# big-nacho/patolette

Hardware: AMD Instinct MI355X
Metric: Mpixels/sec quantized (256-color ICtCp + KMeans) at 1 GPU; palette ΔE vs ref (higher is better)
Workload: dtype f64

## Files before the change

include/patolette_amd.h:

```cpp
#ifndef PATOLETTE_AMD_H
#define PATOLETTE_AMD_H

#include <stddef.h>
#include <stdint.h>

#include "patolette.h"

#ifdef __cplusplus
extern "C" {
#endif

int  patolette_amd_device_count(void);
int  patolette_amd_set_device(int ordinal);
const char *patolette_amd_last_error(void);
void *patolette_amd_malloc(size_t bytes);
void patolette_amd_free(void *dptr);
int  patolette_amd_memcpy_h2d(void *dst, const void *src, size_t bytes);
int  patolette_amd_memcpy_d2h(void *dst, const void *src, size_t bytes);
int  patolette_amd_synchronize(void);
void patolette_amd_release_workspace(void);
int  patolette_amd_fill_image(double *d_planar, size_t n, uint64_t seed);
int  patolette_amd_fill_weights(double *d_weights, size_t n, uint64_t seed);

void patolette_amd_device(size_t width, size_t height, const double *d_data, const double *d_weights,
// ... 155 lines not shown
} patolette_amd__Comm;
void patolette_amd_slice(size_t total_pixels, size_t slice_begin, size_t slice_pixels, const double *slice_data,
                         const double *slice_weights, size_t palette_size, const patolette__QuantizationOptions *options,
                         const patolette_amd__Comm *comm, double *palette, size_t *slice_map, int *exit_code);
void patolette_amd_slice_device(size_t total_pixels, size_t slice_begin, size_t slice_pixels, const double *d_slice_data,
                                const double *d_slice_weights, size_t palette_size, const patolette__QuantizationOptions *options,
                                const patolette_amd__Comm *comm, double *palette, void *d_slice_map, int map_elem_bytes,
                                int *exit_code);
int patolette_amd_set_invariant_sums(int on);
int patolette_amd_set_kmeans_update(int mode);

int patolette_amd_set_split_loop(int mode);
int patolette_amd_set_global_quantiser(int on_device);

int patolette_amd_set_subsample_cache(int on);

int patolette_amd_subsample_indices(size_t n, size_t take, int32_t *out);
int patolette_amd_eigen_sym3(const double a_colmajor[9], double w[3], double z[9]);
int patolette_amd_principal_axis(const double cov6[6], double axis[3]);
int patolette_amd_eigen_sym3_device(const double *a_colmajor, size_t count, double *w, double *z, int *info);
int patolette_amd_debug_gq_table(const double *table, const uint32_t *counts, int weighted, size_t palette_size, int route, int *kbase, int *error,
                                 int *cuts, unsigned char *bucket_table, uint64_t *begin, uint64_t *n, double *sw, double *mean,
                                 uint64_t *prefix_w0, double *prefix, int *cut_table);
int patolette_amd_pow(const double *x, double y, double *out, size_t n);

enum {
    PAMD_SRGB_TO_ICTCP = 0,
    PAMD_SRGB_TO_CIELUV = 1,
    PAMD_ICTCP_TO_REC2020 = 2,
    PAMD_CIELUV_TO_REC2020 = 3,
    PAMD_SRGB_TO_REC2020 = 4,
    PAMD_REC2020_TO_SRGB = 5,
    PAMD_CIELUV_TO_ICTCP = 6
};
int patolette_amd_convert(int which, double *planar, size_t n);

int patolette_amd_quantize_clusters(const double *colors, const double *weights, size_t n, size_t K,
                                    double *centers, size_t *n_clusters);

int patolette_amd_kmeans_refine(const double *colors, const double *weights, size_t n,
                                double *centers_io, size_t k, int niter, size_t max_samples);
int patolette_amd_debug_km_route(void);

int patolette_amd_nn_map(const double *colors, size_t n, const double *palette, size_t k, size_t *map);
int patolette_amd_debug_nn_route(int route);
int patolette_amd_debug_nn_map_elem(const double *colors, size_t n, const double *palette, size_t k, int map_elem_bytes, int misalign,
// ... 66 lines not shown
```

patolette_amd/_native.py:

```python
import ctypes as C
import os

HERE = os.path.dirname(os.path.abspath(__file__))
LIB_PATH = os.path.join(HERE, "lib", "libpatolette_amd.so")

dp = C.POINTER(C.c_double)
zp = C.POINTER(C.c_size_t)


class QuantizationOptions(C.Structure):
    _fields_ = [("dither", C.c_bool), ("palette_only", C.c_bool), ("color_space", C.c_int),
                ("kmeans_niter", C.c_int), ("kmeans_max_samples", C.c_size_t), ("verbose", C.c_bool)]


class Stats(C.Structure):
    _fields_ = [(n, C.c_double) for n in ("ms_total", "ms_upload", "ms_convert", "ms_gq", "ms_lq",
                                          "ms_kmeans", "ms_map", "ms_download", "ms_saliency")] + \
               [(n, C.c_size_t) for n in ("n_base_clusters", "n_clusters", "split_evals", "split_px",
                                          "lq_rounds", "kmeans_samples", "dither_segments", "dither_repairs",
                                          "dither_rounds", "dither_through", "dither_jumps", "dither_solo")]

    def as_dict(self):
        return {n: getattr(self, n) for n, _ in self._fields_}

# ... 32 lines not shown
    "patolette_amd_last_error": (C.c_char_p, []),
    "patolette_amd_malloc": (C.c_void_p, [C.c_size_t]),
    "patolette_amd_free": (None, [C.c_void_p]),
    "patolette_amd_memcpy_h2d": (C.c_int, [C.c_void_p, C.c_void_p, C.c_size_t]),
    "patolette_amd_memcpy_d2h": (C.c_int, [C.c_void_p, C.c_void_p, C.c_size_t]),
    "patolette_amd_synchronize": (C.c_int, []),
    "patolette_amd_release_workspace": (None, []),
    "patolette_amd_batch_dmap": (None, [C.c_size_t, C.c_size_t, C.c_size_t, C.POINTER(C.c_void_p), C.c_int, C.POINTER(dp), C.c_double,
                                        C.c_size_t, C.POINTER(QuantizationOptions), C.POINTER(dp), C.c_void_p, C.c_int,
                                        C.POINTER(C.c_int)]),
    "patolette_amd_slice": (None, [C.c_size_t, C.c_size_t, C.c_size_t, dp, dp, C.c_size_t, C.POINTER(QuantizationOptions),
                                   C.POINTER(Comm), dp, zp, C.POINTER(C.c_int)]),
    "patolette_amd_slice_device": (None, [C.c_size_t, C.c_size_t, C.c_size_t, C.c_void_p, C.c_void_p, C.c_size_t,
                                          C.POINTER(QuantizationOptions), C.POINTER(Comm), dp, C.c_void_p, C.c_int, C.POINTER(C.c_int)]),
    "patolette_amd_set_invariant_sums": (C.c_int, [C.c_int]),
    "patolette_amd_set_kmeans_update": (C.c_int, [C.c_int]),
    "patolette_amd_set_subsample_cache": (C.c_int, [C.c_int]),
    "patolette_amd_subsample_indices": (C.c_int, [C.c_size_t, C.c_size_t, C.POINTER(C.c_int32)]),
    "patolette_amd_eigen_sym3": (C.c_int, [dp, dp, dp]),
    "patolette_amd_principal_axis": (C.c_int, [dp, dp]),
    "patolette_amd_eigen_sym3_device": (C.c_int, [dp, C.c_size_t, dp, dp, C.POINTER(C.c_int)]),
    "patolette_amd_debug_gq_table": (C.c_int, [dp, C.c_void_p, C.c_int, C.c_size_t, C.c_int, C.POINTER(C.c_int), C.POINTER(C.c_int), C.c_void_p,
                                               C.c_void_p, C.c_void_p, C.c_void_p, dp, dp, C.c_void_p, dp, C.c_void_p]),
    "patolette_amd_fill_image": (C.c_int, [C.c_void_p, C.c_size_t, C.c_uint64]),
    "patolette_amd_fill_weights": (C.c_int, [C.c_void_p, C.c_size_t, C.c_uint64]),
    "patolette_amd_device": (None, [C.c_size_t, C.c_size_t, C.c_void_p, C.c_void_p, C.c_size_t,
                                    C.POINTER(QuantizationOptions), dp, C.c_void_p, C.c_int, C.POINTER(C.c_int)]),
    "patolette_amd_quantize": (None, [C.c_size_t, C.c_size_t, dp, dp, C.c_double, C.c_size_t, C.POINTER(QuantizationOptions), dp, zp,
                                      C.POINTER(C.c_int)]),
    "patolette_amd_quantize_rows": (None, [C.c_size_t, C.c_size_t, dp, dp, C.c_double, C.c_size_t, C.POINTER(QuantizationOptions), dp,
                                           zp, C.POINTER(C.c_int)]),
    "patolette_amd_saliency_weights": (C.c_int, [C.c_size_t, C.c_size_t, dp, C.c_double, dp]),
    "patolette_amd_mbd": (C.c_int, [C.c_size_t, C.c_size_t, C.POINTER(C.c_float), C.c_int, C.POINTER(C.c_float)]),
    **_pair("patolette_amd_u8", None, [C.c_size_t, C.c_size_t, C.c_void_p, C.c_int, C.c_void_p, C.c_double, C.c_size_t,
                                       C.POINTER(QuantizationOptions), dp, C.c_void_p, C.c_void_p, C.c_int, C.c_void_p, C.POINTER(C.c_int)]),
    **_pair("patolette_amd_frames_u8", None, [C.c_size_t, C.c_size_t, C.c_size_t, C.c_void_p, C.c_int, C.c_void_p, C.c_double, C.c_size_t,
                                              C.POINTER(QuantizationOptions), dp, C.c_void_p, C.c_void_p, C.c_int, C.c_void_p,
                                              C.POINTER(C.c_int)]),
    **_pair("patolette_amd_remap_u8", None, [C.c_size_t, C.c_size_t, C.c_size_t, C.c_void_p, C.c_int, dp, C.c_void_p, C.c_size_t, C.c_int,
                                             C.c_void_p, C.c_int, C.c_void_p, C.POINTER(C.c_int)]),
    **_pair("patolette_amd_remap_ordered_u8", None, [C.c_size_t, C.c_size_t, C.c_size_t, C.c_void_p, C.c_int, dp, C.c_void_p, C.c_size_t,
                                                     C.c_double, C.c_void_p, C.c_int, C.c_void_p, C.POINTER(C.c_int)]),
    "patolette_amd_debug_remap_two_pass": (C.c_int, [C.c_int]),
    **_pair("patolette_amd_remap_rgba_u8", None, [C.c_size_t, C.c_size_t, C.c_size_t, C.c_void_p, C.c_int, dp, C.c_void_p, C.c_size_t, C.c_int,
                                                  C.c_int, C.c_double, C.c_void_p, C.c_int, C.c_void_p, C.POINTER(C.c_int)]),
    "patolette_amd_debug_rgba_stamp_quad": (C.c_int, [C.c_int]),
# ... 87 lines not shown
def last_error():
    return lib().patolette_amd_last_error().decode("utf-8", "replace")


def last_stats():
    s = Stats()
    lib().patolette_amd_last_stats(C.byref(s))
    return s.as_dict()


def last_split_trace():
    hdr = SplitTrace()
    n = lib().patolette_amd_last_split_trace(C.byref(hdr), None, 0)
    recs = (SplitRecord * max(1, n))()
    lib().patolette_amd_last_split_trace(C.byref(hdr), recs, n)
    return dict(n_base=hdr.n_base, n_clusters=hdr.n_clusters, stopped_early=bool(hdr.stopped_early),
                gq_axis=[float(v) for v in hdr.gq_axis], gq_cov6=[float(v) for v in hdr.gq_cov6],
                gq_cuts=[int(v) for v in hdr.gq_cuts][:hdr.n_base + 1],
                splits=[dict(row=r.row, new_row=r.new_row, split=r.split, degenerate=r.degenerate, n=r.n, n_left=r.n_left,
                             n_right=r.n_right, sw=r.sw, axis=[float(v) for v in r.axis], cov6=[float(v) for v in r.cov6],
                             dist=r.dist, dist_left=r.dist_left, dist_right=r.dist_right, benefit=r.benefit) for r in recs[:n]])


def debug_gq_table(table, counts, weighted, palette_size, route, details=True):
    import numpy as np
    nq = 14 if weighted else 10
    t = np.ascontiguousarray(table, dtype=np.float64).reshape(-1)
    c = np.ascontiguousarray(counts, dtype=np.uint32).reshape(-1)
    if t.size != nq * 2 * 512 or c.size != 512:
        raise ValueError("debug_gq_table: table must hold %d x 2 x 512 doubles and counts 512 entries" % nq)
    kbase, error = C.c_int(0), C.c_int(0)
    cuts = np.zeros(14, dtype=np.int32)
    lut = np.zeros(512, dtype=np.uint8)
    begin, n = np.zeros(12, dtype=np.uint64), np.zeros(12, dtype=np.uint64)
    sw, mean = np.zeros(12), np.zeros((12, 3))
    pw0 = np.zeros((2, 513), dtype=np.uint64) if details else None
    pre = np.zeros((14, 513)) if details else None
    ctab = np.zeros((13, 513), dtype=np.int32) if details else None
    vp = lambda a: a.ctypes.data_as(C.c_void_p) if a is not None else None
    rc = lib().patolette_amd_debug_gq_table(t.ctypes.data_as(dp), vp(c), 1 if weighted else 0, int(palette_size), int(route), C.byref(kbase),
                                            C.byref(error), vp(cuts), vp(lut), vp(begin), vp(n), sw.ctypes.data_as(dp), mean.ctypes.data_as(dp),
                                            vp(pw0), pre.ctypes.data_as(dp) if details else None, vp(ctab))
    if rc != 0:
        raise RuntimeError("patolette_amd_debug_gq_table: %d (%s)" % (rc, last_error()))
    k = kbase.value
    out = dict(kbase=k, error=error.value, cuts=[int(v) for v in cuts[:k + 1]] if k else [], bucket_table=lut, begin=begin[:k].copy(),
# ... 32 lines not shown
```

patolette_amd/csrc/pipeline.hip:

```cpp
#include <algorithm>
#include <functional>
#include <chrono>
#include <cmath>
#include <atomic>
#include <memory>
#include <mutex>
#include <thread>
#include <future>
#include <type_traits>

#include "color_device.h"
#include "common.h"
#include "host_math.h"
#include "kmeans.h"
#include "map.h"
#include "ordered.h"
#include "delta.h"
#include "measure.h"
#include "lzw.h"
#include "lzw_near.h"
#include "hist.h"
#include "saliency.h"
#include "quant.h"
#include "rgba.h"
// ... 818 lines not shown

struct Engine {
    int device = -1;
    hipStream_t stream = nullptr;
    const Shard *shard = nullptr;
    bool invariant = false;
    DevBuf<unsigned char> commbuf;
    PinBuf<unsigned char> h_comm;
    DevBuf<int> shard_ids;
    PinBuf<float> h_cent;
    PinBuf<ConvertStats> h_cstats;
    hipEvent_t ev_stats = nullptr;
    hipStream_t stream2 = nullptr;
    hipEvent_t ev_up[2] = {nullptr, nullptr}, ev_join = nullptr;
    size_t prep_N = 0, prep_planes = 0;
    DevBuf<double> src, wsrc, cvt, bufA, bufB, aux;
    DevBuf<unsigned short> bkt;
    DevBuf<NodeDev> nodes;
    DevBuf<NodeIn> stage_in;
    DevBuf<NodeOut> stage_out;
    DevBuf<int> ids, round_nodes, node_tile0;
    DevBuf<Tile> tilesA, tilesP;
    DevBuf<double> hist, sum6, dpal;
    DevBuf<unsigned long long> hsize, tileoff;
    DevBuf<unsigned int> hcount, tilecnt;
    DevBuf<unsigned char> lut, dmap, src8, pal8, quant8;
    DevBuf<unsigned char> dl_maps, dl_shown;
    DevBuf<unsigned long long> dl_words, dl_masks;
    DevBuf<unsigned long long> ms_words;
    DevBuf<MeasureTile> ms_tiles;
    DevBuf<unsigned> ms_p8;
    DevBuf<LzwFrame> lz_frames;
    DevBuf<unsigned> lz_stage, lz_bits, lz_out;
    DevBuf<unsigned long long> lz_gbit, lz_words;
    DevBuf<unsigned char> lz_near;
    DevBuf<unsigned> rgba_cnt;
    DevBuf<int> rgba_cpos;
    DevBuf<unsigned char> rgba_rgb, rgba_map;
    DevBuf<double> rgba_w;
    PinBuf<unsigned> h_rgba_m;
    DevBuf<unsigned> rr_words;
    PinBuf<unsigned> h_rr_words;
    DevBuf<unsigned long long> hs_units, hs_words, hs_counts;
    DevBuf<unsigned> hs_tiles;
    DevBuf<unsigned char> hs_rgb;
    DevBuf<double> hs_w;
// ... 279 lines not shown
    E.hist.reserve(z.hist, file, line); E.hsize.reserve(z.hsize, file, line); E.hcount.reserve(z.hcount, file, line); E.lut.reserve(z.lut, file, line);
}

static void gq_prepare(Engine &E, size_t N, bool weighted) {
    hipStream_t s = E.stream;
    const size_t planes = weighted ? 4 : 3;
    const QuantSizes z(N, planes, 1);
    reserve_quant_tables(E, z);
    const int ntA = (int)z.tilesA, ntP = (int)z.tilesP;
    E.h_round.reserve(kBuckets);
    E.round_nodes.reserve(1); E.node_tile0.reserve(2);
    const size_t hs = hist_slot_doubles();
    hipLaunchKernelGGL(k_gq_prepare, 64, 256, 0, s, E.tilesA.p, ntA, E.tilesP.p, ntP, (unsigned long long)N, E.round_nodes.p, E.node_tile0.p,
                       E.hist.p, (unsigned long long)hs, E.hsize.p, E.hcount.p);
    HIP_CHECK(hipGetLastError());
    E.prep_N = N; E.prep_planes = planes;
}



std::atomic<int> g_lq_device{getenv("PAMD_LQ_DEVICE") ? atoi(getenv("PAMD_LQ_DEVICE")) : 2};
std::atomic<int> g_gq_device{getenv("PAMD_GQ_DEVICE") ? atoi(getenv("PAMD_GQ_DEVICE")) : 1};
constexpr size_t kLqDeviceAutoPixels = (size_t)40 << 20;

static bool lq_device_eligible(const Engine &E, size_t N, size_t K, bool verbose, bool allow_device) {
    const int lq_mode = g_lq_device.load(std::memory_order_relaxed);
    return allow_device && (lq_mode == 1 || (lq_mode == 2 && N < kLqDeviceAutoPixels)) && !E.shard && !verbose && K <= (size_t)kLqDevMaxK;
}

static void ws_prepare(Engine &E, size_t N, size_t K, bool weighted, bool verbose) {
    const size_t planes = weighted ? 4 : 3;
    const bool lq_dev = lq_device_eligible(E, N, K, verbose, true);
    E.cvt.reserve(planes * N); E.cstats.reserve(1);
    reserve_quant_tables(E, QuantSizes(N, planes, lq_dev ? (size_t)kLqRoundCap : 1));
    E.round_nodes.reserve(1); E.node_tile0.reserve(2); E.h_round.reserve(kBuckets);
    E.nodes.reserve(std::max<size_t>(4 * K + 64, lq_dev ? (size_t)kLqNodeCap : 0));
    E.h_dbl.reserve(16 * kBuckets * 2 + 64);
    E.gq.reserve(1); E.gqout.reserve(1); E.h_gqout.reserve(1); E.h_gq.reserve(1);
    const size_t nput = kGqMaxK + 1;
    E.stage_in.reserve(nput); E.stage_out.reserve(nput); E.ids.reserve(nput); E.h_stage_in.reserve(nput); E.h_stage_out.reserve(nput);
    E.h_ids.reserve(nput); E.h_ids_get.reserve(nput);
    E.h_cent.reserve(3 * K);
    E.dpal.reserve(3 * K); E.h_pal.reserve(3 * K);
    if (lq_dev) { E.lqctl.reserve(1); E.h_lqhead.reserve(1); E.h_lqrec.reserve(kLqNodeCap); E.h_lqcen.reserve(kLqNodeCap); }
}

// ... 201 lines not shown
    }
}

static bool gq_root_histogram(QuantCall &C) {
    Engine &E = C.E;
    hipStream_t s = E.stream;
    const HNode &root = C.hn[0];
    if (!node_axis(root, C.axis)) return false;
    E.trace.clear();
    E.trace_pending = false;
    E.trace_hdr = patolette_amd__SplitTrace{};
    for (int j = 0; j < 3; j++) E.trace_hdr.gq_axis[j] = C.axis[j];
    for (int q = 0; q < 6; q++) E.trace_hdr.gq_cov6[q] = root.cov6[q] / root.sw;
    {
        NodeIn d = make_nodedev(root, C.bnd);
        for (int j = 0; j < 3; j++) d.axis[j] = C.axis[j];
        d.slot = 0;
        put_nodes(E, {0}, {d});
    }
    launch_minmax(C.qroot, E.tilesA.p, C.ntA0, C.N, E.nodes.p, s, C.mom_path);
    if (C.sh) shard_exchange_keys(E, shard_upload_ids(E, {0}), 1);
    launch_hist(C.qroot, true, E.tilesA.p, C.ntA0, C.N, E.nodes.p, E.hist.p, E.hsize.p, E.hcount.p, s, !C.mom_path, C.Nt >= ((size_t)1 << 18));
    if (C.sh) { comm_sum_dev(E, E.hist.p, C.hs, 0); comm_sum_dev(E, E.hcount.p, kBuckets, 2); }
    return true;
}

static void gq_trace_header(Engine &E) {
    const GqOut &o = *E.h_gqout.p;
    E.trace_hdr.n_base = o.kbase;
    for (int j = 0; j <= o.kbase && j < 14; j++) E.trace_hdr.gq_cuts[j] = (size_t)o.cuts[j];
}

static int finish_device_loop(QuantCall &C, int kbase, int first_base, int nnodes) {
    Engine &E = C.E;
    if (kbase >= 0) E.stats.n_base_clusters = (size_t)kbase;
    E.stats.ms_gq = now_ms() - C.t0;
    C.t0 = now_ms();
    const int rc = lq_device_loop(E, C.N, C.K, C.weighted, C.inv_sums, C.bnd, C.qlq, kbase, first_base, nnodes, C.centers, C.len, C.max_members);
    if (kbase < 0) {
        gq_trace_header(E);
        E.stats.n_base_clusters = (size_t)E.h_gqout.p->kbase;
    }
    if (rc != 0) return rc;
    E.stats.n_clusters = C.len;
    E.trace_hdr.n_clusters = (int32_t)C.len; E.trace_hdr.n_records = (int32_t)E.lq_commits.size();
    E.cluster_centers = C.centers;
// ... 2657 lines not shown
}

int patolette_amd_debug_fault(int which) { return g_debug_fault.exchange(which); }
int patolette_amd_debug_workspace(int flags) { return g_debug_ws.exchange(flags & (kWsPoison | kWsCount | kWsLog)); }
unsigned long long patolette_amd_debug_late_growths(void) { return g_late_growths.load(); }
int patolette_amd_set_split_loop(int mode) { return g_lq_device.exchange(mode < 0 || mode > 2 ? 2 : mode); }
int patolette_amd_set_global_quantiser(int on_device) { return g_gq_device.exchange(on_device ? 1 : 0); }
void patolette_amd_dither_config(int segments, int warm) { dither_config(segments, warm); }
void patolette_amd_dither_layout(int lanes) { dither_layout(lanes); }
int patolette_amd_debug_dither_solo_cap(int cap) { return dither_solo_cap(cap); }
int patolette_amd_debug_dither_stall_passes(int n) { return dither_stall_passes(n); }
int patolette_amd_dither_layout_in_use(size_t width, size_t height, size_t k) { return dither_lane_layout(width, height, (int)k) ? 1 : 0; }
int patolette_amd_debug_dither_lane_tables(double *geom30, float *amb3, unsigned char *tables, size_t capacity) {
    return guarded([&](Engine &E) -> int { return dither_lane_tables(E.nn, geom30, amb3, tables, capacity, E.stream); });
}
void patolette_amd_last_stats(patolette_amd__Stats *out) { *out = engine().stats; }
size_t patolette_amd_last_split_trace(patolette_amd__SplitTrace *hdr, patolette_amd__SplitRecord *recs, size_t capacity) {
    Engine &E = engine();
    try { materialise_trace(E); } catch (const std::exception &e) { E.last_error = e.what(); E.trace.clear(); }
    if (hdr) *hdr = E.trace_hdr;
    if (recs) std::memcpy(recs, E.trace.data(), sizeof *recs * std::min(capacity, E.trace.size()));
    return E.trace.size();
}
size_t patolette_amd_last_cluster_centers(double *out, size_t capacity_rows) {
    Engine &E = engine();
    const size_t len = E.cluster_centers.size() / 3;
    if (out && len <= capacity_rows)
        for (int j = 0; j < 3; j++) for (size_t i = 0; i < len; i++) out[(size_t)j * capacity_rows + i] = E.cluster_centers[(size_t)j * len + i];
    return len;
}
size_t patolette_amd_last_map_palette(double *out, size_t capacity_rows) {
    const std::vector<double> &mp = engine().map_palette;
    const size_t len = mp.size() / 3;
    if (out && capacity_rows >= len)
        for (int j = 0; j < 3; j++) for (size_t i = 0; i < len; i++) out[(size_t)j * capacity_rows + i] = mp[(size_t)j * len + i];
    return len;
}

void patolette_amd_profile_enable(int on) {
    KernelTimer &t = ktimer();
    if (engine().stream) (void)hipStreamSynchronize(engine().stream);
    t.reset();
    t.enabled = on != 0;
}
void patolette_amd_profile_only(const char *kernel_name) { ktimer().only = kernel_name ? kernel_name : ""; ktimer().only_seen = 0; }
void patolette_amd_profile_sample(int period) { ktimer().sample_period = period > 1 ? (unsigned)period : 1u; }
// ... 13 lines not shown
```

patolette_amd/csrc/quant.hip:

```cpp
#include "quant.h"

#include <atomic>

#include <type_traits>

namespace pamd {

template <typename T>
__device__ __forceinline__ T block_scan_incl(T v, T *smem) {
    const int lane = threadIdx.x & 63, wid = threadIdx.x >> 6, nw = blockDim.x >> 6;
#pragma unroll
    for (int o = 1; o < 64; o <<= 1) {
        T t = __shfl_up(v, o, 64);
        if (lane >= o) v += t;
    }
    __syncthreads();
    if (lane == 63) smem[wid] = v;
    __syncthreads();
    if (wid == 0) {
        T s = lane < nw ? smem[lane] : T(0);
#pragma unroll
        for (int o = 1; o < 16; o <<= 1) {
            T t = __shfl_up(s, o, 64);
            if (lane >= o) s += t;
// ... 104 lines not shown
            mn = fmin(mn, d); mx = fmax(mx, d);
        }
    }
    for (; i < t.count; i += 256) {
        size_t p = t.start + i;
        double d = project(px[p], py[p], pz[p], a0, a1, a2);
        mn = fmin(mn, d); mx = fmax(mx, d);
    }
#pragma unroll
    for (int o = 32; o > 0; o >>= 1) { mn = fmin(mn, __shfl_down(mn, o, 64)); mx = fmax(mx, __shfl_down(mx, o, 64)); }
    __shared__ double smn[4], smx[4];
    if ((threadIdx.x & 63) == 0) { smn[threadIdx.x >> 6] = mn; smx[threadIdx.x >> 6] = mx; }
    __syncthreads();
    if (threadIdx.x == 0) {
        for (int w = 1; w < 4; w++) { mn = fmin(mn, smn[w]); mx = fmax(mx, smx[w]); }
        if (mn <= mx) {
            atomicMin(&nd.minkey[blockIdx.x & (kSlots - 1)], f64_key(mn));
            atomicMax(&nd.maxkey[blockIdx.x & (kSlots - 1)], f64_key(mx));
        }
    }
}

constexpr int kHistCombineMin = 12;
template <bool W, bool GQ>
__global__ __launch_bounds__(512) void k_hist(QuantBuffers qb, const Tile *__restrict__ tiles, int ntiles, NodeDev *nodes,
                                              double *hist, unsigned long long *hsize, unsigned int *hcount, const int from_end,
                                              const RoundDyn *__restrict__ dyn) {
    constexpr int NQ = GQ ? (W ? 14 : 10) : (W ? 4 : 3);
    int nblk = (int)gridDim.x;
    if (dyn) {
        ntiles = dyn->ntA;
        nblk = min(ntiles, nblk);
        if ((int)blockIdx.x >= nblk) return;
    }
    constexpr int NQS = GQ ? kNQ_GQ : kNQ_LQ;
    extern __shared__ double lds[];
    double *h = lds;
    unsigned long long *siz = (unsigned long long *)(h + NQ * 2 * kBuckets);
    unsigned int *cnt = (unsigned int *)(siz + kBuckets);
    for (int i = threadIdx.x; i < NQ * 2 * kBuckets; i += blockDim.x) h[i] = 0.0;
    for (int i = threadIdx.x; i < kBuckets; i += blockDim.x) { cnt[i] = 0u; siz[i] = 0ULL; }
    __syncthreads();

    const int per = (ntiles + nblk - 1) / nblk;
    const int bid = from_end ? nblk - 1 - (int)blockIdx.x : (int)blockIdx.x;
    const int tfirst = bid * per, tlast = min(ntiles, tfirst + per);
// ... 107 lines not shown
    const int e1 = (int)((__double_as_longlong(k.M1) >> 52) & 0x7ff) - 1023 - 52;
    const int B = e0 - e1, E = e0 + B;
    const int F = 2 * B < 45 ? 2 * B : 45;
    FixK f;
    f.magic = ldexp(1.5, 52 + E - F); f.s = F - B; f.ghi = ldexp(1.0, e0); f.glo = ldexp(1.0, E - F);
    return f;
}
__device__ __forceinline__ long long fix_quant(const double v, const double magic) {
    return __double_as_longlong(v + magic) - __double_as_longlong(magic);
}
template <bool W, bool GQ>
__global__ __launch_bounds__(512) void k_hist_fix(QuantBuffers qb, const Tile *__restrict__ tiles, int ntiles, NodeDev *nodes,
                                              double *hist, unsigned long long *hsize, unsigned int *hcount, const int from_end) {
    constexpr int NQ = GQ ? (W ? 14 : 10) : (W ? 4 : 3);
    constexpr int NQS = GQ ? kNQ_GQ : kNQ_LQ;
    extern __shared__ unsigned long long lds64[];
    unsigned long long *h = lds64;
    unsigned long long *siz = h + NQ * kBuckets;
    unsigned int *cnt = (unsigned int *)(siz + kBuckets);
    for (int i = threadIdx.x; i < NQ * kBuckets; i += blockDim.x) h[i] = 0ULL;
    for (int i = threadIdx.x; i < kBuckets; i += blockDim.x) { cnt[i] = 0u; siz[i] = 0ULL; }
    __syncthreads();

    const int per = (ntiles + (int)gridDim.x - 1) / (int)gridDim.x;
    const int bid = from_end ? (int)gridDim.x - 1 - (int)blockIdx.x : (int)blockIdx.x;
    const int tfirst = bid * per, tlast = min(ntiles, tfirst + per);
    int since_flush = 0;
    for (int ti = tfirst; ti < tlast; ti++) {
        const Tile t = tiles[ti];
        NodeDev &nd = nodes[t.node];
        const double a0 = nd.axis[0], a1 = nd.axis[1], a2 = nd.axis[2];
        double mn, mx;
        node_minmax(nd, mn, mx);
        const bool degenerate = (mx - mn < kDelta);
        const double sc = 1 / (mx - mn);
        const FixK flin = make_fixk(nd.klin), fquad = make_fixk(nd.kquad);
        const double *px = qb.buf[nd.buf], *py = px + qb.N, *pz = py + qb.N, *pw = pz + qb.N;
        const unsigned long long gslot0 = nd.gslot0;
        if (threadIdx.x == 0) nd.degenerate = degenerate ? 1 : 0;

        auto one = [&](const size_t p, const double x, const double y, const double z, const double w) {
            unsigned b;
            if (degenerate) {
                b = (unsigned)((p - nd.begin + gslot0) % kBuckets);
            } else {
                double ratio = (project(x, y, z, a0, a1, a2) - mn) * sc;
                unsigned long long bq = (unsigned long long)((double)kBuckets * ratio);
                b = bq < (unsigned long long)(kBuckets - 1) ? (unsigned)bq : (unsigned)(kBuckets - 1);
            }
            qb.bkt[p] = (unsigned short)b;
            double pv[NQ], pm[NQ];
#define HPART(q, val, K) pv[q] = (val); pm[q] = (K).magic
            if constexpr (!GQ) {
                HPART(0, x * w, flin); HPART(1, y * w, flin); HPART(2, z * w, flin);
                if constexpr (W) { HPART(3, w, flin); }
            } else {
                HPART(0, x, flin); HPART(1, y, flin); HPART(2, z, flin);
                HPART(3, (x * x + y * y) + z * z, fquad);
                HPART(4, x * x, fquad); HPART(5, x * y, fquad); HPART(6, y * y, fquad);
                HPART(7, x * z, fquad); HPART(8, y * z, fquad); HPART(9, z * z, fquad);
                if constexpr (W) { HPART(10, x * w, flin); HPART(11, y * w, flin); HPART(12, z * w, flin); HPART(13, w, flin); }
            }
#undef HPART
            unsigned long long wi = 0ULL;
            if constexpr (W && !GQ) wi = (unsigned long long)w;
            bool direct = true;
            if (__ballot(true) == ~0ULL) {
                unsigned long long left = ~0ULL;
#pragma unroll 1
                for (int g = 0; g < 3 && left != 0ULL; g++) {
                    const int first = __builtin_ctzll(left);
                    const unsigned b0 = (unsigned)__builtin_amdgcn_readlane((int)b, first);
                    const bool mine = direct && b == b0;
                    const unsigned long long m = __ballot(mine);
                    if (__popcll(m) < kHistCombineMin) break;
#pragma unroll
                    for (int k2 = 0; k2 < NQ; k2++) {
                        const double vq = (pv[k2] + pm[k2]) - pm[k2];
                        const double sum = wave_sum_dpp63(mine ? vq : 0.0);
                        if ((threadIdx.x & 63) == 63) atomicAdd(&h[k2 * kBuckets + b0], (unsigned long long)fix_quant(sum, pm[k2]));
                    }
                    if constexpr (W && !GQ) {
                        unsigned long long sw2 = mine ? wi : 0ULL;
#pragma unroll
                        for (int o = 32; o > 0; o >>= 1) sw2 += __shfl_down(sw2, o, 64);
                        if ((threadIdx.x & 63) == 0) atomicAdd(&siz[b0], sw2);
                    }
                    if ((threadIdx.x & 63) == 0) atomicAdd(&cnt[b0], (unsigned)__popcll(m));
                    if (mine) direct = false;
                    left &= ~m;
                }
            }
            if (direct) {
                atomicAdd(&cnt[b], 1u);
#pragma unroll
                for (int k2 = 0; k2 < NQ; k2++) atomicAdd(&h[k2 * kBuckets + b], (unsigned long long)fix_quant(pv[k2], pm[k2]));
                if constexpr (W && !GQ) atomicAdd(&siz[b], wi);
            }
        };
        unsigned i = threadIdx.x;
        for (; i + 512 < t.count; i += 1024) {
            const size_t p0 = t.start + i, p1 = p0 + 512;
            const double x0 = px[p0], y0 = py[p0], z0 = pz[p0], x1 = px[p1], y1 = py[p1], z1 = pz[p1];
            double w0 = 1.0, w1 = 1.0;
            if constexpr (W) { w0 = pw[p0]; w1 = pw[p1]; }
            one(p0, x0, y0, z0, w0);
            one(p1, x1, y1, z1, w1);
        }
        for (; i < t.count; i += 512) {
            const size_t p = t.start + i;
            double w = 1.0;
            if constexpr (W) w = pw[p];
            one(p, px[p], py[p], pz[p], w);
        }
        since_flush++;
        const bool flush = (ti + 1 == tlast) || tiles[ti + 1].node != t.node || since_flush >= 16;
        if (!flush) continue;
        since_flush = 0;
        __syncthreads();
        const size_t slot = (size_t)nd.slot;
        double *gh = hist + slot * (size_t)(NQS * 2 * kBuckets);
        for (int i2 = threadIdx.x; i2 < NQ * kBuckets; i2 += blockDim.x) {
            const long long S = (long long)h[i2];
            if (S != 0) {
                const int q = i2 / kBuckets, bb = i2 % kBuckets;
                const bool quad = GQ && q >= 3 && q <= 9;
                const FixK &f = quad ? fquad : flin;
                const long long Sh = (S + (1LL << (f.s - 1))) >> f.s, Sl = S - (Sh << f.s);
                if (Sh != 0) unsafeAtomicAdd(&gh[(q * 2 + 0) * kBuckets + bb], (double)Sh * f.ghi);
                if (Sl != 0) unsafeAtomicAdd(&gh[(q * 2 + 1) * kBuckets + bb], (double)Sl * f.glo);
                h[i2] = 0ULL;
            }
        }
        for (int b = threadIdx.x; b < kBuckets; b += blockDim.x) {
            unsigned c = cnt[b];
            if (c) { atomicAdd(&hcount[slot * kBuckets + b], c); cnt[b] = 0u; }
            if constexpr (W && !GQ) { const unsigned long long s2 = siz[b]; if (s2) { atomicAdd(&hsize[slot * kBuckets + b], s2); siz[b] = 0ULL; } }
        }
        __syncthreads();
    }
}

template <bool W>
__global__ __launch_bounds__(512) void k_cut(NodeDev *nodes, const int *__restrict__ round_nodes, const double *__restrict__ hist,
                                             const unsigned long long *__restrict__ hsize, const unsigned int *__restrict__ hcount,
                                             unsigned char *lut, const int fault, const RoundDyn *__restrict__ dyn) {
    if (dyn && (int)blockIdx.x >= dyn->nr) return;
    __shared__ double sd[4 * 16];
    __shared__ unsigned long long su[2 * 16];
    __shared__ double best_v[8];
    __shared__ int best_i[8];
    __shared__ double tot[8];
    __shared__ unsigned long long tots[2];
    __shared__ int s_split;
    const int b = threadIdx.x;
    NodeDev &nd = nodes[round_nodes[blockIdx.x]];
    const size_t slot = (size_t)nd.slot;
    const double *gh = hist + slot * (size_t)(kNQ_LQ * 2 * kBuckets);
    constexpr int NQ = W ? 4 : 3;
    double p[NQ][2];
// ... 194 lines not shown
#pragma unroll
            for (int q = 0; q < 8; q++) sum += v[q];
        }
        const unsigned long long inc = block_scan_incl<unsigned long long>(sum, su);
        if (threadIdx.x == blockDim.x - 1) total = inc;
        unsigned long long run = base + inc - sum;
        for (int g = a; g < b; g += 8) {
            unsigned v[8];
#pragma unroll
            for (int q = 0; q < 8; q++) v[q] = g + q < b ? tilecnt[(size_t)(g + q) * kMaxChildren + k] : 0u;
#pragma unroll
            for (int q = 0; q < 8; q++) {
                if (g + q < b) tileoff[(size_t)(g + q) * kMaxChildren + k] = run;
                run += v[q];
            }
        }
        if (threadIdx.x == 0) nd.cbegin[k] = base;
        __syncthreads();
        base += total;
        __syncthreads();
    }
    if (threadIdx.x == 0) nd.cbegin[nch] = base;
}

template <bool W>
__global__ __launch_bounds__(256, 5) void k_scatter(QuantBuffers qb, const Tile *__restrict__ tiles, int ntiles, NodeDev *nodes,
                                                    const unsigned char *__restrict__ lut, const unsigned long long *__restrict__ tileoff,
                                                    const int from_end) {
    constexpr int R = kTileP / 256;
    __shared__ unsigned long long off[R][4][kMaxChildren];
    const int lane = threadIdx.x & 63, wid = threadIdx.x >> 6;
    const unsigned long long ltmask = (1ULL << lane) - 1ULL;
    if ((from_end & 4) && nodes[0].nchild == 2) return;
    const int per = (ntiles + (int)gridDim.x - 1) / (int)gridDim.x;
    const int bid = (from_end & 1) ? (int)gridDim.x - 1 - (int)blockIdx.x : (int)blockIdx.x;
    const int tfirst = bid * per, tlast = min(ntiles, tfirst + per);
    for (int ti = tfirst; ti < tlast; ti++) {
        const Tile t = tiles[ti];
        const NodeDev &nd = nodes[t.node];
        const unsigned char *l = lut + (size_t)nd.slot * kBuckets;
        const int nch = nd.nchild;
        unsigned cr[R];
#pragma unroll
        for (int r = 0; r < R; r++) {
            unsigned i = r * 256 + threadIdx.x;
            int ch = 255;
// ... 250 lines not shown
    if (g < 1) g = 1;
    KTIME("k_sum3", s, 24.0 * N);
    hipLaunchKernelGGL(k_sum3, (int)g, 256, 0, s, planar, N, k, d_out6);
    HIP_CHECK(hipGetLastError());
}

void launch_minmax(const QuantBuffers &qb, const Tile *d_tiles, int ntiles, size_t px, NodeDev *d_nodes, hipStream_t s, bool from_end,
                   const RoundDyn *dyn, const double *px_src, const RoundLists *lists) {
    if (!ntiles) return;
    KTIME_DYN("k_minmax", s, 24.0, px, px_src);
    if (dyn && lists) hipLaunchKernelGGL(k_minmax<true>, ntiles, 256, 0, s, qb, d_tiles, d_nodes, from_end ? 1 : 0, dyn, *lists);
    else hipLaunchKernelGGL(k_minmax<false>, ntiles, 256, 0, s, qb, d_tiles, d_nodes, from_end ? 1 : 0, dyn, RoundLists{});
    HIP_CHECK(hipGetLastError());
}

template <bool W>
static void launch_hist_fix(const QuantBuffers &qb, const Tile *d_tiles, int ntiles, size_t px, NodeDev *d_nodes, double *d_hist,
                            unsigned long long *d_hsize, unsigned int *d_hcount, hipStream_t s, bool from_end) {
    constexpr int NQ = W ? 14 : 10;
    const size_t lds = (size_t)NQ * kBuckets * sizeof(unsigned long long) + kBuckets * (sizeof(unsigned int) + sizeof(unsigned long long));
    static PerDeviceOnce attr_set;
    attr_set.once([&] { HIP_CHECK(hipFuncSetAttribute((const void *)k_hist_fix<W, true>, hipFuncAttributeMaxDynamicSharedMemorySize, (int)lds)); });
    KTIME("k_hist_gq", s, (W ? 34.0 : 26.0) * px);
    const int g = std::min(ntiles, 256 * (W ? 2 : 3));
    hipLaunchKernelGGL((k_hist_fix<W, true>), g, 512, lds, s, qb, d_tiles, ntiles, d_nodes, d_hist, d_hsize, d_hcount, from_end ? 1 : 0);
    HIP_CHECK(hipGetLastError());
}

template <bool W, bool GQ>
static void launch_hist_t(const QuantBuffers &qb, const Tile *d_tiles, int ntiles, size_t px, NodeDev *d_nodes, double *d_hist,
                          unsigned long long *d_hsize, unsigned int *d_hcount, hipStream_t s, bool from_end,
                          const RoundDyn *dyn = nullptr, const double *px_src = nullptr) {
    constexpr int NQ = GQ ? (W ? 14 : 10) : (W ? 4 : 3);
    size_t lds = (size_t)NQ * 2 * kBuckets * sizeof(double) + kBuckets * (sizeof(unsigned int) + sizeof(unsigned long long));
    static PerDeviceOnce attr_set;
    attr_set.once([&] { HIP_CHECK(hipFuncSetAttribute((const void *)k_hist<W, GQ>, hipFuncAttributeMaxDynamicSharedMemorySize, (int)lds)); });
    KTIME_DYN(GQ ? "k_hist_gq" : "k_hist_lq", s, (W ? 34.0 : 26.0), px, px_src);
    const int g = std::min(ntiles, 256 * (GQ ? 1 : 4));
    hipLaunchKernelGGL((k_hist<W, GQ>), g, 512, lds, s, qb, d_tiles, ntiles, d_nodes, d_hist, d_hsize, d_hcount, from_end ? 1 : 0, dyn);
    HIP_CHECK(hipGetLastError());
}

__global__ __launch_bounds__(512) void k_gq_prefix(const double *__restrict__ hist, const unsigned int *__restrict__ hcount, GqDpDev *g) {
    __shared__ double sh[4][kBuckets + 1];
    __shared__ unsigned long long sc[kBuckets + 1];
    const int b = threadIdx.x;
#pragma unroll
// ... 80 lines not shown
    else { if (gq) launch_hist_t<false, true>(qb, d_tiles, ntiles, px, d_nodes, d_hist, d_hsize, d_hcount, s, from_end);
           else launch_hist_t<false, false>(qb, d_tiles, ntiles, px, d_nodes, d_hist, d_hsize, d_hcount, s, from_end, dyn, px_src); }
}

std::atomic<int> g_debug_fault{0};
void launch_cut(bool weighted, NodeDev *d_nodes, const int *d_round_nodes, int nround, const double *d_hist,
                const unsigned long long *d_hsize, const unsigned int *d_hcount, unsigned char *d_lut, hipStream_t s, const RoundDyn *dyn, const double *nr_src) {
    if (!nround) return;
    KTIME_DYN("k_cut", s, (double)kNQ_LQ * 2 * kBuckets * 8, nround, nr_src);
    const int fault = g_debug_fault.load(std::memory_order_relaxed);
    if (weighted) hipLaunchKernelGGL(k_cut<true>, nround, 512, 0, s, d_nodes, d_round_nodes, d_hist, d_hsize, d_hcount, d_lut, fault, dyn);
    else hipLaunchKernelGGL(k_cut<false>, nround, 512, 0, s, d_nodes, d_round_nodes, d_hist, d_hsize, d_hcount, d_lut, fault, dyn);
    HIP_CHECK(hipGetLastError());
}

void launch_partition(const QuantBuffers &qb, const Tile *d_ptiles, int nptiles, size_t px, const int *d_round_nodes,
                      const int *d_node_tile0, int nround, NodeDev *d_nodes, const unsigned char *d_lut,
                      unsigned int *d_tilecnt, unsigned long long *d_tileoff, bool fuse_cov, hipStream_t s, bool invariant, bool from_end,
                      const RoundDyn *dyn, const double *px_src, bool gated) {
    const int fe = (from_end ? 1 : 0) | (gated ? 2 : 0);
    if (!nround) return;
    if (nptiles) { KTIME_DYN("k_count", s, 2.0, px, px_src); hipLaunchKernelGGL(k_count, nptiles, 256, 0, s, qb, d_ptiles, d_nodes, d_lut, d_tilecnt, fe & 1, dyn); }
    { KTIME_DYN("k_scan", s, 12.0 * kMaxChildren / (double)kTileP, dyn ? px : (size_t)nptiles * kTileP, px_src);
      hipLaunchKernelGGL(k_scan, nround, 1024, 0, s, d_round_nodes, d_node_tile0, d_nodes, d_tilecnt, d_tileoff, dyn); }
    if (nptiles) {
        KTIME_DYN(fuse_cov ? "k_scatter_cov" : "k_scatter", s, (qb.weighted ? 66.0 : 50.0), px, px_src);
        if (fuse_cov) {
            const int gb = std::min(nptiles, 256 * ((invariant || qb.weighted) ? 2 : 3));
            const bool nt = 2 * (size_t)(qb.weighted ? 4 : 3) * qb.N * sizeof(double) > kInfinityCacheBytes;
            auto go = [&](auto kernel) {
                hipLaunchKernelGGL(kernel, gb, 256, 0, s, qb, d_ptiles, nptiles, d_nodes, (const NodeDev *)d_nodes, d_tileoff, fe, dyn);
            };
            if (invariant) {
                if (qb.weighted) { if (nt) go(k_scatter_bin<true, true, true>); else go(k_scatter_bin<true, true, false>); }
                else { if (nt) go(k_scatter_bin<false, true, true>); else go(k_scatter_bin<false, true, false>); }
            } else if (qb.weighted) { if (nt) go(k_scatter_bin<true, false, true>); else go(k_scatter_bin<true, false, false>); }
            else { if (nt) go(k_scatter_bin<false, false, true>); else go(k_scatter_bin<false, false, false>); }
            if (gated) {
                HIP_CHECK(hipGetLastError());
                const int fg = (from_end ? 1 : 0) | 4;
                if (qb.weighted) hipLaunchKernelGGL((k_scatter<true>), nptiles, 256, 0, s, qb, d_ptiles, nptiles, d_nodes, d_lut, d_tileoff, fg);
                else hipLaunchKernelGGL((k_scatter<false>), nptiles, 256, 0, s, qb, d_ptiles, nptiles, d_nodes, d_lut, d_tileoff, fg);
            }
        } else {
            if (qb.weighted) hipLaunchKernelGGL((k_scatter<true>), nptiles, 256, 0, s, qb, d_ptiles, nptiles, d_nodes, d_lut, d_tileoff, fe);
            else hipLaunchKernelGGL((k_scatter<false>), nptiles, 256, 0, s, qb, d_ptiles, nptiles, d_nodes, d_lut, d_tileoff, fe);
        }
// ... 24 lines not shown
```

Baseline: 3121.

## Split GQ histogram tiles into sub-units, pre-add magic, parallel root scan

```diff
diff --git a/include/patolette_amd.h b/include/patolette_amd.h
--- a/include/patolette_amd.h
+++ b/include/patolette_amd.h
@@ -201,6 +201,8 @@
 int patolette_amd_debug_gq_table(const double *table, const uint32_t *counts, int weighted, size_t palette_size, int route, int *kbase, int *error,
                                  int *cuts, unsigned char *bucket_table, uint64_t *begin, uint64_t *n, double *sw, double *mean,
                                  uint64_t *prefix_w0, double *prefix, int *cut_table);
+
+int patolette_amd_debug_last_gq_table(int keep, double *table, uint32_t *counts, size_t capacity_doubles);
 int patolette_amd_pow(const double *x, double y, double *out, size_t n);
 
 enum {
diff --git a/patolette_amd/_native.py b/patolette_amd/_native.py
--- a/patolette_amd/_native.py
+++ b/patolette_amd/_native.py
@@ -78,6 +78,7 @@
     "patolette_amd_eigen_sym3_device": (C.c_int, [dp, C.c_size_t, dp, dp, C.POINTER(C.c_int)]),
     "patolette_amd_debug_gq_table": (C.c_int, [dp, C.c_void_p, C.c_int, C.c_size_t, C.c_int, C.POINTER(C.c_int), C.POINTER(C.c_int), C.c_void_p,
                                                C.c_void_p, C.c_void_p, C.c_void_p, dp, dp, C.c_void_p, dp, C.c_void_p]),
+    "patolette_amd_debug_last_gq_table": (C.c_int, [C.c_int, dp, C.c_void_p, C.c_size_t]),
     "patolette_amd_fill_image": (C.c_int, [C.c_void_p, C.c_size_t, C.c_uint64]),
     "patolette_amd_fill_weights": (C.c_int, [C.c_void_p, C.c_size_t, C.c_uint64]),
     "patolette_amd_device": (None, [C.c_size_t, C.c_size_t, C.c_void_p, C.c_void_p, C.c_size_t,
@@ -211,6 +212,19 @@
                              dist=r.dist, dist_left=r.dist_left, dist_right=r.dist_right, benefit=r.benefit) for r in recs[:n]])
 
 
+def debug_keep_gq_table(on):
+    return lib().patolette_amd_debug_last_gq_table(1 if on else 0, None, None, 0)
+
+
+def debug_last_gq_table():
+    import numpy as np
+    table, counts = np.zeros((14, 2, 512)), np.zeros(512, dtype=np.uint32)
+    rows = lib().patolette_amd_debug_last_gq_table(1, table.ctypes.data_as(dp), counts.ctypes.data_as(C.c_void_p), table.size)
+    if rows < 0:
+        raise RuntimeError("patolette_amd_debug_last_gq_table: no table kept (%s)" % last_error())
+    return table, counts
+
+
 def debug_gq_table(table, counts, weighted, palette_size, route, details=True):
     import numpy as np
     nq = 14 if weighted else 10
diff --git a/patolette_amd/csrc/pipeline.hip b/patolette_amd/csrc/pipeline.hip
--- a/patolette_amd/csrc/pipeline.hip
+++ b/patolette_amd/csrc/pipeline.hip
@@ -864,6 +864,9 @@
     DevBuf<int> ids, round_nodes, node_tile0;
     DevBuf<Tile> tilesA, tilesP;
     DevBuf<double> hist, sum6, dpal;
+    DevBuf<double> dbg_gq_table;
+    DevBuf<unsigned int> dbg_gq_counts;
+    size_t dbg_gq_doubles = 0;
     DevBuf<unsigned long long> hsize, tileoff;
     DevBuf<unsigned int> hcount, tilecnt;
     DevBuf<unsigned char> lut, dmap, src8, pal8, quant8;
@@ -1189,6 +1192,7 @@
 std::atomic<int> g_lq_device{getenv("PAMD_LQ_DEVICE") ? atoi(getenv("PAMD_LQ_DEVICE")) : 2};
 std::atomic<int> g_gq_device{getenv("PAMD_GQ_DEVICE") ? atoi(getenv("PAMD_GQ_DEVICE")) : 1};
 constexpr size_t kLqDeviceAutoPixels = (size_t)40 << 20;
+std::atomic<int> g_keep_gq_table{0};
 
 static bool lq_device_eligible(const Engine &E, size_t N, size_t K, bool verbose, bool allow_device) {
     const int lq_mode = g_lq_device.load(std::memory_order_relaxed);
@@ -1436,6 +1440,13 @@
     if (C.sh) shard_exchange_keys(E, shard_upload_ids(E, {0}), 1);
     launch_hist(C.qroot, true, E.tilesA.p, C.ntA0, C.N, E.nodes.p, E.hist.p, E.hsize.p, E.hcount.p, s, !C.mom_path, C.Nt >= ((size_t)1 << 18));
     if (C.sh) { comm_sum_dev(E, E.hist.p, C.hs, 0); comm_sum_dev(E, E.hcount.p, kBuckets, 2); }
+    if (g_keep_gq_table.load(std::memory_order_relaxed)) {
+        E.sync();
+        E.dbg_gq_table.reserve(C.hs); E.dbg_gq_counts.reserve(kBuckets);
+        HIP_CHECK(hipMemcpyAsync(E.dbg_gq_table.p, E.hist.p, C.hs * sizeof(double), hipMemcpyDeviceToDevice, s));
+        HIP_CHECK(hipMemcpyAsync(E.dbg_gq_counts.p, E.hcount.p, kBuckets * sizeof(unsigned int), hipMemcpyDeviceToDevice, s));
+        E.dbg_gq_doubles = C.hs;
+    }
     return true;
 }
 
@@ -4139,6 +4150,19 @@
     if (recs) std::memcpy(recs, E.trace.data(), sizeof *recs * std::min(capacity, E.trace.size()));
     return E.trace.size();
 }
+int patolette_amd_debug_last_gq_table(int keep, double *table, uint32_t *counts, size_t capacity_doubles) {
+    const int prev = g_keep_gq_table.exchange(keep ? 1 : 0);
+    if (!table && !counts) return prev;
+    try {
+        Engine &E = engine();
+        if (!E.dbg_gq_doubles || !table || !counts || capacity_doubles < E.dbg_gq_doubles) return -1;
+        HIP_CHECK(hipSetDevice(E.device));
+        E.sync();
+        HIP_CHECK(hipMemcpy(table, E.dbg_gq_table.p, E.dbg_gq_doubles * sizeof(double), hipMemcpyDeviceToHost));
+        HIP_CHECK(hipMemcpy(counts, E.dbg_gq_counts.p, kBuckets * sizeof(uint32_t), hipMemcpyDeviceToHost));
+        return (int)(E.dbg_gq_doubles / (2 * kBuckets));
+    } catch (const std::exception &) { return -1; }
+}
 size_t patolette_amd_last_cluster_centers(double *out, size_t capacity_rows) {
     Engine &E = engine();
     const size_t len = E.cluster_centers.size() / 3;
diff --git a/patolette_amd/csrc/quant.hip b/patolette_amd/csrc/quant.hip
--- a/patolette_amd/csrc/quant.hip
+++ b/patolette_amd/csrc/quant.hip
@@ -150,6 +150,7 @@
 }
 
 constexpr int kHistCombineMin = 12;
+constexpr int kHistSub = 4;
 template <bool W, bool GQ>
 __global__ __launch_bounds__(512) void k_hist(QuantBuffers qb, const Tile *__restrict__ tiles, int ntiles, NodeDev *nodes,
                                               double *hist, unsigned long long *hsize, unsigned int *hcount, const int from_end,
@@ -303,12 +304,16 @@
     for (int i = threadIdx.x; i < kBuckets; i += blockDim.x) { cnt[i] = 0u; siz[i] = 0ULL; }
     __syncthreads();
 
-    const int per = (ntiles + (int)gridDim.x - 1) / (int)gridDim.x;
+    const int nunits = ntiles * kHistSub;
+    const int per = (nunits + (int)gridDim.x - 1) / (int)gridDim.x;
     const int bid = from_end ? (int)gridDim.x - 1 - (int)blockIdx.x : (int)blockIdx.x;
-    const int tfirst = bid * per, tlast = min(ntiles, tfirst + per);
+    const int ufirst = bid * per, ulast = min(nunits, ufirst + per);
+    const int tfirst = ufirst / kHistSub, tlast = (ulast + kHistSub - 1) / kHistSub;
     int since_flush = 0;
     for (int ti = tfirst; ti < tlast; ti++) {
         const Tile t = tiles[ti];
+        const unsigned plo = ti == tfirst ? (unsigned)(ufirst - ti * kHistSub) * (unsigned)(kTileA / kHistSub) : 0u;
+        const unsigned phi = min(t.count, (unsigned)min(ulast - ti * kHistSub, kHistSub) * (unsigned)(kTileA / kHistSub));
         NodeDev &nd = nodes[t.node];
         const double a0 = nd.axis[0], a1 = nd.axis[1], a2 = nd.axis[2];
         double mn, mx;
@@ -330,8 +335,8 @@
                 b = bq < (unsigned long long)(kBuckets - 1) ? (unsigned)bq : (unsigned)(kBuckets - 1);
             }
             qb.bkt[p] = (unsigned short)b;
-            double pv[NQ], pm[NQ];
-#define HPART(q, val, K) pv[q] = (val); pm[q] = (K).magic
+            double pa[NQ], pm[NQ];
+#define HPART(q, val, K) pa[q] = (val) + (K).magic; pm[q] = (K).magic
             if constexpr (!GQ) {
                 HPART(0, x * w, flin); HPART(1, y * w, flin); HPART(2, z * w, flin);
                 if constexpr (W) { HPART(3, w, flin); }
@@ -346,7 +351,8 @@
             unsigned long long wi = 0ULL;
             if constexpr (W && !GQ) wi = (unsigned long long)w;
             bool direct = true;
-            if (__ballot(true) == ~0ULL) {
+            if (__ballot(true) == ~0ULL &&
+                __popcll(__ballot(b == (unsigned)__builtin_amdgcn_readfirstlane((int)b))) >= kHistCombineMin) {
                 unsigned long long left = ~0ULL;
 #pragma unroll 1
                 for (int g = 0; g < 3 && left != 0ULL; g++) {
@@ -357,9 +363,11 @@
                     if (__popcll(m) < kHistCombineMin) break;
 #pragma unroll
                     for (int k2 = 0; k2 < NQ; k2++) {
-                        const double vq = (pv[k2] + pm[k2]) - pm[k2];
+                        const double vq = pa[k2] - pm[k2];
                         const double sum = wave_sum_dpp63(mine ? vq : 0.0);
-                        if ((threadIdx.x & 63) == 63) atomicAdd(&h[k2 * kBuckets + b0], (unsigned long long)fix_quant(sum, pm[k2]));
+                        if ((threadIdx.x & 63) == 63)
+                            atomicAdd(&h[k2 * kBuckets + b0], (unsigned long long)fix_quant(sum, pm[k2]) +
+                                                              (unsigned long long)__popcll(m) * (unsigned long long)__double_as_longlong(pm[k2]));
                     }
                     if constexpr (W && !GQ) {
                         unsigned long long sw2 = mine ? wi : 0ULL;
@@ -375,12 +383,12 @@
             if (direct) {
                 atomicAdd(&cnt[b], 1u);
 #pragma unroll
-                for (int k2 = 0; k2 < NQ; k2++) atomicAdd(&h[k2 * kBuckets + b], (unsigned long long)fix_quant(pv[k2], pm[k2]));
+                for (int k2 = 0; k2 < NQ; k2++) atomicAdd(&h[k2 * kBuckets + b], (unsigned long long)__double_as_longlong(pa[k2]));
                 if constexpr (W && !GQ) atomicAdd(&siz[b], wi);
             }
         };
-        unsigned i = threadIdx.x;
-        for (; i + 512 < t.count; i += 1024) {
+        unsigned i = plo + threadIdx.x;
+        for (; i + 512 < phi; i += 1024) {
             const size_t p0 = t.start + i, p1 = p0 + 512;
             const double x0 = px[p0], y0 = py[p0], z0 = pz[p0], x1 = px[p1], y1 = py[p1], z1 = pz[p1];
             double w0 = 1.0, w1 = 1.0;
@@ -388,7 +396,7 @@
             one(p0, x0, y0, z0, w0);
             one(p1, x1, y1, z1, w1);
         }
-        for (; i < t.count; i += 512) {
+        for (; i < phi; i += 512) {
             const size_t p = t.start + i;
             double w = 1.0;
             if constexpr (W) w = pw[p];
@@ -401,22 +409,25 @@
         __syncthreads();
         const size_t slot = (size_t)nd.slot;
         double *gh = hist + slot * (size_t)(NQS * 2 * kBuckets);
-        for (int i2 = threadIdx.x; i2 < NQ * kBuckets; i2 += blockDim.x) {
-            const long long S = (long long)h[i2];
-            if (S != 0) {
-                const int q = i2 / kBuckets, bb = i2 % kBuckets;
-                const bool quad = GQ && q >= 3 && q <= 9;
-                const FixK &f = quad ? fquad : flin;
-                const long long Sh = (S + (1LL << (f.s - 1))) >> f.s, Sl = S - (Sh << f.s);
-                if (Sh != 0) unsafeAtomicAdd(&gh[(q * 2 + 0) * kBuckets + bb], (double)Sh * f.ghi);
-                if (Sl != 0) unsafeAtomicAdd(&gh[(q * 2 + 1) * kBuckets + bb], (double)Sl * f.glo);
-                h[i2] = 0ULL;
-            }
-        }
-        for (int b = threadIdx.x; b < kBuckets; b += blockDim.x) {
-            unsigned c = cnt[b];
-            if (c) { atomicAdd(&hcount[slot * kBuckets + b], c); cnt[b] = 0u; }
-            if constexpr (W && !GQ) { const unsigned long long s2 = siz[b]; if (s2) { atomicAdd(&hsize[slot * kBuckets + b], s2); siz[b] = 0ULL; } }
+        for (int bb = threadIdx.x; bb < kBuckets; bb += blockDim.x) {
+            const unsigned c32 = cnt[bb];
+            const unsigned long long c = c32;
+            if (c32) {
+#pragma unroll
+                for (int q = 0; q < NQ; q++) {
+                    const bool quad = GQ && q >= 3 && q <= 9;
+                    const FixK &f = quad ? fquad : flin;
+                    const long long S = (long long)(h[q * kBuckets + bb] - c * (unsigned long long)__double_as_longlong(f.magic));
+                    h[q * kBuckets + bb] = 0ULL;
+                    if (S == 0) continue;
+                    const long long Sh = (S + (1LL << (f.s - 1))) >> f.s, Sl = S - (Sh << f.s);
+                    if (Sh != 0) unsafeAtomicAdd(&gh[(q * 2 + 0) * kBuckets + bb], (double)Sh * f.ghi);
+                    if (Sl != 0) unsafeAtomicAdd(&gh[(q * 2 + 1) * kBuckets + bb], (double)Sl * f.glo);
+                }
+                atomicAdd(&hcount[slot * kBuckets + bb], c32);
+                cnt[bb] = 0u;
+            }
+            if constexpr (W && !GQ) { const unsigned long long s2 = siz[bb]; if (s2) { atomicAdd(&hsize[slot * kBuckets + bb], s2); siz[bb] = 0ULL; } }
         }
         __syncthreads();
     }
@@ -657,6 +668,57 @@
     }
     if (threadIdx.x == 0) nd.cbegin[nch] = base;
 }
+constexpr int kScanGroup = 64;
+__global__ __launch_bounds__(256) void k_scan_root(const int *__restrict__ round_nodes, const int *__restrict__ node_tile0, NodeDev *nodes,
+                                                   const unsigned int *__restrict__ tilecnt, unsigned long long *tileoff) {
+    static_assert(kMaxChildren % 4 == 0, "a tile's counts are read four children at a time");
+    __shared__ unsigned long long part[4][8];
+    __shared__ unsigned long long before[kMaxChildren], total[kMaxChildren];
+    NodeDev &nd = nodes[round_nodes[0]];
+    const int t0 = node_tile0[0], t1 = node_tile0[1];
+    const int first = t0 + (int)blockIdx.x * kScanGroup;
+    const int nch = nd.nchild;
+    const int lane = threadIdx.x & 63, wid = threadIdx.x >> 6;
+    for (int c0 = 0; c0 < nch; c0 += 4) {
+        unsigned long long s[8] = {0, 0, 0, 0, 0, 0, 0, 0};
+#pragma unroll 4
+        for (int t = t0 + (int)threadIdx.x; t < t1; t += 256) {
+            const uint4 v = *reinterpret_cast<const uint4 *>(tilecnt + (size_t)t * kMaxChildren + c0);
+            const bool pre = t < first;
+            s[4] += v.x; s[5] += v.y; s[6] += v.z; s[7] += v.w;
+            s[0] += pre ? v.x : 0u; s[1] += pre ? v.y : 0u; s[2] += pre ? v.z : 0u; s[3] += pre ? v.w : 0u;
+        }
+#pragma unroll
+        for (int i = 0; i < 8; i++) {
+#pragma unroll
+            for (int o = 32; o > 0; o >>= 1) s[i] += __shfl_down(s[i], o, 64);
+        }
+        if (lane == 0) {
+#pragma unroll
+            for (int i = 0; i < 8; i++) part[wid][i] = s[i];
+        }
+        __syncthreads();
+        if (threadIdx.x < 8) {
+            const unsigned long long sum = part[0][threadIdx.x] + part[1][threadIdx.x] + part[2][threadIdx.x] + part[3][threadIdx.x];
+            if (threadIdx.x < 4) before[c0 + threadIdx.x] = sum; else total[c0 + threadIdx.x - 4] = sum;
+        }
+        __syncthreads();
+    }
+    const int t = first + lane;
+    for (int k = wid; k < nch; k += 4) {
+        unsigned long long base = nd.begin;
+        for (int j = 0; j < k; j++) base += total[j];
+        const unsigned v = t < t1 ? tilecnt[(size_t)t * kMaxChildren + k] : 0u;
+        const unsigned incl = wave_scan_incl_u32(v);
+        if (t < t1) tileoff[(size_t)t * kMaxChildren + k] = base + before[k] + (unsigned long long)(incl - v);
+        if (blockIdx.x == 0 && lane == 0) nd.cbegin[k] = base;
+    }
+    if (blockIdx.x == 0 && threadIdx.x == 0) {
+        unsigned long long base = nd.begin;
+        for (int j = 0; j < nch; j++) base += total[j];
+        nd.cbegin[nch] = base;
+    }
+}
 
 template <bool W>
 __global__ __launch_bounds__(256, 5) void k_scatter(QuantBuffers qb, const Tile *__restrict__ tiles, int ntiles, NodeDev *nodes,
@@ -953,7 +1015,9 @@
     static PerDeviceOnce attr_set;
     attr_set.once([&] { HIP_CHECK(hipFuncSetAttribute((const void *)k_hist_fix<W, true>, hipFuncAttributeMaxDynamicSharedMemorySize, (int)lds)); });
     KTIME("k_hist_gq", s, (W ? 34.0 : 26.0) * px);
-    const int g = std::min(ntiles, 256 * (W ? 2 : 3));
+    const int slots = 256 * 2, nunits = ntiles * kHistSub;
+    const int per = ntiles <= slots ? kHistSub : (nunits + slots - 1) / slots;
+    const int g = (nunits + per - 1) / per;
     hipLaunchKernelGGL((k_hist_fix<W, true>), g, 512, lds, s, qb, d_tiles, ntiles, d_nodes, d_hist, d_hsize, d_hcount, from_end ? 1 : 0);
     HIP_CHECK(hipGetLastError());
 }
@@ -1080,7 +1144,9 @@
     if (!nround) return;
     if (nptiles) { KTIME_DYN("k_count", s, 2.0, px, px_src); hipLaunchKernelGGL(k_count, nptiles, 256, 0, s, qb, d_ptiles, d_nodes, d_lut, d_tilecnt, fe & 1, dyn); }
     { KTIME_DYN("k_scan", s, 12.0 * kMaxChildren / (double)kTileP, dyn ? px : (size_t)nptiles * kTileP, px_src);
-      hipLaunchKernelGGL(k_scan, nround, 1024, 0, s, d_round_nodes, d_node_tile0, d_nodes, d_tilecnt, d_tileoff, dyn); }
+      if (nround == 1 && !dyn && nptiles > kScanGroup)
+          hipLaunchKernelGGL(k_scan_root, (nptiles + kScanGroup - 1) / kScanGroup, 256, 0, s, d_round_nodes, d_node_tile0, d_nodes, d_tilecnt, d_tileoff);
+      else hipLaunchKernelGGL(k_scan, nround, 1024, 0, s, d_round_nodes, d_node_tile0, d_nodes, d_tilecnt, d_tileoff, dyn); }
     if (nptiles) {
         KTIME_DYN(fuse_cov ? "k_scatter_cov" : "k_scatter", s, (qb.weighted ? 66.0 : 50.0), px, px_src);
         if (fuse_cov) {
```

Result: no change. 3136, median of 6 (+0.5%).
